# Fadi987/PL-BERT

Measured on AMD Instinct MI355X. Metric: phoneme-tokens/sec, higher is better.
Workload: dtype bf16; 1 GPU; PL-BERT masked-phoneme training step (fwd+loss+bwd+allreduce+AdamW), ALBERT hidden 768 / 12 shared layers / FFN 2048 / 12 heads, seq_len 512, batch 32 per GPU; global_batch=32, seq_len=512, parallelism=dp1

## Files before the change

include/plbert.h:

```cpp
#ifndef PLBERT_H
#define PLBERT_H

#include <stdint.h>

#ifdef __cplusplus
extern "C" {
#endif

typedef struct PlbEngine PlbEngine;

typedef struct {
  int32_t vocab_size;
  int32_t embedding_size;
  int32_t hidden_size;
  int32_t num_attention_heads;
  int32_t intermediate_size;
  int32_t num_hidden_layers;
  int32_t max_position_embeddings;
  int32_t type_vocab_size;
  float layer_norm_eps;
  int32_t num_phonemes;
  int32_t num_tokens;
  int32_t max_batch;
  int32_t max_seq;
// ... 210 lines not shown
int plb_profile_num_classes(void);
const char* plb_profile_class_name(int cls);
int plb_profile_read(double* ms, int64_t* launches, double* flops, double* bytes);

void plb_debug_skip_piece(int index);
void plb_debug_ln_fault(int mode, int launches);
int plb_debug_hb_audit(PlbEngine* e, int32_t on, int32_t break_wait);
int plb_debug_hb_report(const PlbEngine* e, int64_t* checks, int32_t* violations, char* first, int32_t first_bytes);
int plb_comm_trace(PlbEngine* e, int32_t on);
int plb_comm_trace_read(PlbEngine* e, int32_t max_pieces, int32_t* n, int64_t* begin, int64_t* end, float* released_ms,
                        float* done_ms, float* tail_ms);
void plb_set_gemm_nt_tile(int tile);
void plb_set_gemm_nt_prefetch(int on);
void plb_set_attn_bwd_fused(int on);
void plb_set_prune_last(int on);

#ifdef __cplusplus
}
#endif
#endif
```

plbert_amd/_lib.py:

```python
from __future__ import annotations

import ctypes as C
import os

import torch

HERE = os.path.dirname(os.path.abspath(__file__))
LIB_PATH = os.environ.get("PLBERT_HIP_LIB") or os.path.join(HERE, "libplbert_hip.so")

PLB_PARAM_NAMES = [
    "encoder.embeddings.word_embeddings.weight",
    "encoder.embeddings.position_embeddings.weight",
    "encoder.embeddings.token_type_embeddings.weight",
    "encoder.embeddings.LayerNorm.weight",
    "encoder.embeddings.LayerNorm.bias",
    "encoder.encoder.embedding_hidden_mapping_in.weight",
    "encoder.encoder.embedding_hidden_mapping_in.bias",
    "encoder.encoder.albert_layer_groups.0.albert_layers.0.full_layer_layer_norm.weight",
    "encoder.encoder.albert_layer_groups.0.albert_layers.0.full_layer_layer_norm.bias",
    "encoder.encoder.albert_layer_groups.0.albert_layers.0.attention.query.weight",
    "encoder.encoder.albert_layer_groups.0.albert_layers.0.attention.key.weight",
    "encoder.encoder.albert_layer_groups.0.albert_layers.0.attention.value.weight",
    "encoder.encoder.albert_layer_groups.0.albert_layers.0.attention.query.bias",
    "encoder.encoder.albert_layer_groups.0.albert_layers.0.attention.key.bias",
# ... 51 lines not shown


class PlbAttn(C.Structure):
    _fields_ = [
        ("qkv", C.c_void_p), ("ldqkv", C.c_int), ("lengths", C.c_void_p),
        ("B", C.c_int), ("S", C.c_int), ("NH", C.c_int), ("H", C.c_int), ("scale", C.c_float),
        ("ctx", C.c_void_p), ("ldctx", C.c_int), ("lse", C.c_void_p),
        ("dctx", C.c_void_p), ("lddctx", C.c_int), ("delta", C.c_void_p), ("dqkv", C.c_void_p), ("lddqkv", C.c_int),
        ("colpart", C.c_void_p), ("colpart_accumulate", C.c_int),
        ("ctx8", C.c_void_p), ("ldctx8", C.c_int), ("ctx_scale", C.c_void_p), ("ctx_amax", C.c_void_p),
        ("dqkv8", C.c_void_p), ("lddqkv8", C.c_int), ("dqkv_scale", C.c_void_p), ("dqkv_amax", C.c_void_p),
        ("qoff", C.c_void_p), ("q", C.c_void_p), ("ldq", C.c_int), ("nq_total", C.c_int), ("dq", C.c_void_p), ("lddq", C.c_int),
        ("dq8", C.c_void_p), ("lddq8", C.c_int),
        ("row_start", C.c_void_p),
        ("key_words", C.c_void_p), ("ldkw", C.c_int),
    ]


class PlbEmbed(C.Structure):
    _fields_ = [
        ("ids", C.c_void_p), ("T", C.c_int), ("S", C.c_int), ("E", C.c_int), ("V", C.c_int),
        ("word", C.c_void_p), ("pos", C.c_void_p), ("type0", C.c_void_p), ("gamma", C.c_void_p), ("beta", C.c_void_p),
        ("eps", C.c_float), ("out", C.c_void_p), ("ldo", C.c_int), ("dout", C.c_void_p), ("lddo", C.c_int),
        ("dx", C.c_void_p), ("dword", C.c_void_p), ("dpos", C.c_void_p), ("partials", C.c_void_p), ("nblocks", C.c_int),
        ("row_start", C.c_void_p), ("lengths", C.c_void_p), ("B", C.c_int), ("fill_slots", C.c_int),
    ]


class PlbEmbedIn(C.Structure):
    _fields_ = [
# ... 170 lines not shown
    "plb_mask_batch": (i32, [vp, vp, i32, i32, u64, u32, f32, f32, f32, i32, i32, vp, vp, vp, vp, vp]),
    "plb_profile_enable": (None, [i32]),
    "plb_profile_num_classes": (i32, []),
    "plb_profile_class_name": (C.c_char_p, [i32]),
    "plb_profile_read": (i32, [P(f64), P(i64), P(f64), P(f64)]),
    "plb_debug_skip_piece": (None, [i32]),
    "plb_debug_ln_fault": (None, [i32, i32]),
    "plb_debug_hb_audit": (i32, [vp, i32, i32]),
    "plb_debug_hb_report": (i32, [vp, P(i64), P(i32), vp, i32]),
    "plb_comm_trace": (i32, [vp, i32]),
    "plb_comm_trace_read": (i32, [vp, i32, P(i32), P(i64), P(i64), P(f32), P(f32), P(f32)]),
    "plb_set_gemm_nt_tile": (None, [i32]),
    "plb_set_gemm_nt_prefetch": (None, [i32]),
    "plb_set_attn_bwd_fused": (None, [i32]),
    "plb_set_prune_last": (None, [i32]),
}
PUBLIC_SYMBOLS = list(PUBLIC)
INTERNAL = {
    **{name: PUBLIC[name] for name in ("plb_set_gemm_nt_tile", "plb_set_gemm_nt_prefetch", "plb_debug_skip_piece",
                                       "plb_debug_ln_fault", "plb_set_attn_bwd_fused")},
    "plb_prof_begin": (i32, [i32, vp, f64, f64]),
    "plb_prof_end": (None, [i32, vp]),
    "plb_launch_gemm_nt_ln": (i32, [P(PlbGemmNT), i32, vp]),
    "plb_launch_gemm_nt_gelud": (i32, [P(PlbGemmNT), i32, vp]),
    "plb_launch_gemm_nt_fp8": (i32, [P(PlbGemmNT), i32, i32, vp]),
    "plb_launch_gemm_nt_fp8_ln": (i32, [P(PlbGemmNT), i32, i32, vp]),
    "plb_launch_gemm_nt_fp8_gelud": (i32, [P(PlbGemmNT), i32, i32, vp]),
    "plb_gemm_nt_fp8_gelud_tile_rows": (i32, [i32]),
    "plb_ln_fault_take": (i32, []),
    "plb_launch_gemm_nt": (i32, [P(PlbGemmNT), i32, i32, vp]),
# ... 11 lines not shown
    "plb_launch_embed_inputs_scatter": (i32, [P(PlbEmbedIn), vp]),
    "plb_embed_inputs_part_floats": (sz, [i32, i32, i32, i32]),
    "plb_launch_amax": (i32, [vp, i32, sz, i32, i32, vp, vp]),
    "plb_launch_fp8_scales": (i32, [vp, vp, vp, i32, f32, i32, vp]),
    "plb_launch_fp8_scales2": (i32, [vp, vp, vp, i32, f32, i32, i32, f32, vp, i32, vp]),
    "plb_launch_quantize": (i32, [vp, i32, sz, i32, i32, vp, vp, i32, i32, vp]),
    "plb_launch_quantize_multi": (i32, [i32, vp, vp, vp, vp, vp, vp, vp]),
    "plb_launch_ln_fwd": (i32, [P(PlbLayerNorm), vp]),
    "plb_launch_ln_bwd": (i32, [P(PlbLayerNorm), vp]),
    "plb_launch_colsum": (i32, [vp, i32, sz, i32, i32, vp, i32, i32, vp, i32, vp]),
    "plb_launch_copy_cols": (i32, [vp, i32, i32, i32, i32, vp, vp]),
    "plb_launch_pooler": (i32, [vp, i32, i32, i32, vp, vp, vp, vp]),
    "plb_launch_attn_fwd": (i32, [P(PlbAttn), vp]),
    "plb_launch_attn_bwd": (i32, [P(PlbAttn), vp]),
    "plb_launch_attn_bwd_fused": (i32, [P(PlbAttn), vp]),
    "plb_launch_gather_rows": (i32, [vp, i32, vp, i32, i32, i32, vp, i32, vp]),
    "plb_launch_scatter_rows": (i32, [vp, i32, vp, i32, i32, vp, i32, vp]),
    "plb_launch_ce_prepare": (i32, [vp, vp, vp, i32, i32, vp, vp, vp, vp]),
    "plb_launch_ce_prepare_packed": (i32, [vp, vp, vp, i32, i32, vp, vp, vp, vp, vp]),
    "plb_launch_unpack_rows": (i32, [vp, i32, i32, vp, vp, i32, i32, i32, vp, vp]),
    "plb_launch_seed_dy": (i32, [vp, vp, vp, i32, i32, i32, i32, vp, vp]),
    "plb_launch_pooler_bwd": (i32, [vp, i32, vp, i32, i32, i32, vp, vp, vp, vp, vp, vp, vp, vp]),
    "plb_launch_seed_dy_first_rows": (i32, [vp, vp, vp, i32, i32, i32, vp, vp]),
    "plb_launch_attn_probs": (i32, [vp, i32, vp, vp, vp, i32, i32, i32, f32, vp, vp]),
    "plb_launch_attn_probs_masked": (i32, [vp, i32, vp, vp, vp, vp, i32, i32, i32, i32, f32, vp, vp]),
    "plb_launch_key_mask_words": (i32, [vp, vp, i32, i32, vp, i32, vp]),
    "plb_launch_add_row_grad": (i32, [vp, vp, vp, vp, i32, i32, i32, i32, vp, vp]),
    "plb_launch_ce_fwd_bwd": (i32, [vp, i32, i32, vp, vp, i32, i32, vp, vp, i32, vp]),
    "plb_launch_sum_rows": (i32, [vp, i32, vp, vp]),
    "plb_launch_token_ce_combine": (i32, [vp, vp, i32, vp, vp, i32, i32, i32, vp, vp, vp, vp]),
# ... 81 lines not shown
```

plbert_amd/csrc/attn.hip:

```cpp
#include "attn_common.h"
#include <stdlib.h>
#include <string.h>

namespace {

#define ATTN_KM 0
#define ATTN_KERNEL(name) name##_kernel
#include "attn_kernels.h"
#undef ATTN_KM
#undef ATTN_KERNEL
#define ATTN_KM 1
#define ATTN_KERNEL(name) name##_km_kernel
#include "attn_kernels.h"
#undef ATTN_KM
#undef ATTN_KERNEL

}

static int check_attn(const PlbAttn* p) {
  if (p->H != p->NH * 64 || p->S < 1 || p->B < 1) return 1;
  if (p->row_start && !p->lengths) return 1;
  if (p->ldqkv % 8 || p->ldctx % 8) return 1;
  if (p->key_words && (p->S > 2048 || p->ldkw < 2 * ((p->S + 63) / 64) || p->qoff)) return 1;
  return 0;
}

extern "C" int plb_launch_attn_fwd(const PlbAttn* p, hipStream_t stream) {
  if (check_attn(p) || (p->ctx8 && (!p->ctx_scale || p->ldctx8 % 8))) return 1;
  if (p->qoff && (!p->q || p->ldq % 8 || p->nq_total < 0)) return 1;
  dim3 grid(((p->S + 127) / 128) * p->NH * p->B), block(256);
  const double unit = (double)p->B * p->NH * (double)p->S * p->S * 64.0;
  const double io = 2.0 * p->B * p->S * (double)p->H;
  const int tok = plb_prof_begin(PLB_K_ATTN_FWD, stream, 4.0 * unit, 4.0 * io);
  if (p->key_words) hipLaunchKernelGGL(attn_fwd_km_kernel, grid, block, 0, stream, *p);
  else hipLaunchKernelGGL(attn_fwd_kernel, grid, block, 0, stream, *p);
  plb_prof_end(tok, stream);
  return hipGetLastError() == hipSuccess ? 0 : 2;
}

static int g_bwd_fused = -2;
extern "C" void plb_set_attn_bwd_fused(int on) { g_bwd_fused = on < 0 ? -1 : (on > 2 ? 1 : on); }
static int launch_attn_bwd_split(const PlbAttn* p, hipStream_t stream) {
  dim3 grid(((p->S + 127) / 128) * p->NH * p->B), block(256);
  const double unit = (double)p->B * p->NH * (double)p->S * p->S * 64.0;
  const double io = 2.0 * p->B * p->S * (double)p->H;
  int tok = plb_prof_begin(PLB_K_ATTN_BWD_DQ, stream, 4.0 * unit, 6.0 * io);
  if (p->key_words) hipLaunchKernelGGL(attn_bwd_dq_km_kernel, grid, block, 0, stream, *p);
  else hipLaunchKernelGGL(attn_bwd_dq_kernel, grid, block, 0, stream, *p);
  plb_prof_end(tok, stream);
  tok = plb_prof_begin(PLB_K_ATTN_BWD_DKV, stream, 4.0 * unit, 6.0 * io);
  if (p->key_words) hipLaunchKernelGGL(attn_bwd_dkv_km_kernel, grid, block, 0, stream, *p);
  else hipLaunchKernelGGL(attn_bwd_dkv_kernel, grid, block, 0, stream, *p);
  plb_prof_end(tok, stream);
  return hipGetLastError() == hipSuccess ? 0 : 2;
}
static PlbAttn attn_samples(const PlbAttn* p, int b0, int nb) {
  PlbAttn q = *p;
  const size_t t0 = (size_t)b0 * p->S;
  q.B = nb;
// ... 2 lines not shown
  q.dctx = p->dctx + t0 * p->lddctx;
  if (p->dqkv) q.dqkv = p->dqkv + t0 * p->lddqkv;
  if (p->dqkv8) q.dqkv8 = p->dqkv8 + t0 * p->lddqkv8;
  if (p->lengths) q.lengths = p->lengths + b0;
  q.lse = p->lse + (size_t)b0 * p->NH * p->S;
  if (p->delta) q.delta = p->delta + (size_t)b0 * p->NH * p->S;
  if (p->colpart) q.colpart = p->colpart + (size_t)b0 * ((p->S + 127) / 128) * 4 * (3 * p->H);
  if (p->key_words) q.key_words = p->key_words + (size_t)b0 * p->ldkw;
  if (p->row_start) {
    q.row_start = p->row_start + b0;
    q.qkv = p->qkv; q.ctx = p->ctx; q.dctx = p->dctx; q.dqkv = p->dqkv; q.dqkv8 = p->dqkv8;
  }
  return q;
}

extern "C" int plb_launch_attn_bwd(const PlbAttn* p, hipStream_t stream) {
  if (check_attn(p) || p->lddctx % 8 || p->lddqkv % 8 || (!p->dqkv && !p->dqkv8) || (p->dqkv8 && (!p->dqkv_scale || p->lddqkv8 % 8))) return 1;
  if (g_bwd_fused == -2) {
    const char* e = getenv("PLBERT_ATTN_BWD");
    g_bwd_fused = (e && !strcmp(e, "fused")) ? 1 : (e && !strcmp(e, "split")) ? 0 : (e && !strcmp(e, "hybrid")) ? 2 : -1;
  }
  const bool hybrid_on = g_bwd_fused == 2;
  if (p->qoff && (!p->q || p->ldq % 8 || p->nq_total < 0 || (!p->dq && !p->dq8) || (p->dq && p->lddq % 8) || (p->dq8 && p->lddq8 % 8))) return 1;
  const bool can_fuse = p->S <= 512 && !(p->dqkv && p->dqkv8) && !p->qoff && !p->key_words;
  if (!can_fuse || g_bwd_fused == 0) return launch_attn_bwd_split(p, stream);
  if (g_bwd_fused == 1) return plb_launch_attn_bwd_fused(p, stream);
  if (p->S <= 384) return launch_attn_bwd_split(p, stream);
  const int items = p->B * p->NH, rounds = (items + 255) / 256;
  if (items * 10 >= rounds * 256 * 9) return plb_launch_attn_bwd_fused(p, stream);
  const int per_round = 256 / p->NH;
  const int full = per_round > 0 ? (p->B / per_round) : 0;
  const int nb_f = full * per_round, rest = p->B - nb_f;
  if (hybrid_on && full >= 1 && per_round * p->NH * 10 >= 256 * 9 && rest * p->NH <= 160) {
    const PlbAttn a = attn_samples(p, 0, nb_f);
    const int rc = plb_launch_attn_bwd_fused(&a, stream);
    if (rc || rest == 0) return rc;
    const PlbAttn b = attn_samples(p, nb_f, rest);
    return launch_attn_bwd_split(&b, stream);
  }
  return launch_attn_bwd_split(p, stream);
}
```

plbert_amd/csrc/attn_kernels.h:

```cpp
#define KEY_WORDS(kwl_, kt_)                                                                                       \
  uint32_t kw0 = ~0u, kw1 = ~0u;                                                                                   \
  if constexpr (ATTN_KM) {                                                                                              \
    kw0 = (uint32_t)__builtin_amdgcn_readlane((int)(kwl_), 2 * (kt_));                                             \
    kw1 = (uint32_t)__builtin_amdgcn_readlane((int)(kwl_), 2 * (kt_) + 1);                                         \
  }

#ifndef RESCALE_TH
#define RESCALE_TH 8.0f
#endif
#ifndef FWD_WAVES
#define FWD_WAVES 3
#endif
__global__ __launch_bounds__(256, ATTN_KM ? 4 : FWD_WAVES) void ATTN_KERNEL(attn_fwd)(PlbAttn p) {
  __shared__ __attribute__((aligned(16))) bf16_t smem[2][2][64 * 64];
  const int tid = threadIdx.x, lane = tid & 63;
  const int wave = __builtin_amdgcn_readfirstlane(tid >> 6);
  DBG_EARLY_EXIT(p);
  const int QT = (p.S + 127) >> 7;
  const int logical = xcd_remap(blockIdx.x, gridDim.x);
  const int bx = logical % QT, bh = logical / QT;
  const int hd = bh % p.NH, b = bh / p.NH;
  const int S = p.S, H = p.H;
  int len = p.lengths ? p.lengths[b] : S;
  len = len < 1 ? 1 : (len > S ? S : len);
// ... 474 lines not shown
  float* cp = p.colpart ? p.colpart + ((size_t)(b * QT + bx) * 4 + wave) * (3 * H) + hd * 64 : nullptr;
  int lane_e = (int)__builtin_amdgcn_mbcnt_hi(~0u, __builtin_amdgcn_mbcnt_lo(~0u, 0u));
  asm volatile("" : "+v"(lane_e));
  float amax8 = 0.f;
  if (rows_valid > 0) {
    bf16_t* out = p.dqkv ? p.dqkv + (tok0 + key0) * p.lddqkv + hd * 64 : nullptr;
    uint8_t* out8 = p.dqkv8 ? p.dqkv8 + (tok0 + key0) * p.lddqkv8 + hd * 64 : nullptr;
    const float qs8 = p.dqkv8 ? p.dqkv_scale[0] : 1.0f;
    const Out8 ok8 = {out8 ? out8 + H : nullptr, p.lddqkv8, qs8, true}, ov8 = {out8 ? out8 + 2 * H : nullptr, p.lddqkv8, qs8, true};
    const bool accq = p.colpart_accumulate != 0;
    store_transposed<(ATTN_OUT_NT & 4) != 0, true>(dk0, dk1, p.scale, patch, out ? out + H : nullptr, p.lddqkv, rows_valid, lane_e,
                                             cp ? cp + H : nullptr, accq, &ok8, &amax8);
    __builtin_amdgcn_wave_barrier();
    store_transposed<(ATTN_OUT_NT & 4) != 0, true>(dv0, dv1, 1.0f, patch, out ? out + 2 * H : nullptr, p.lddqkv, rows_valid, lane_e,
                                             cp ? cp + 2 * H : nullptr, accq, &ov8, &amax8);
  } else if (cp && !p.colpart_accumulate) {
    cp[H + lane_e] = 0.f;
    cp[2 * H + lane_e] = 0.f;
  }
  if (p.dqkv8 && p.dqkv_amax) {
    amax8 = wave_max(amax8);
    if (lane_e == 0) atomic_max_abs(p.dqkv_amax, amax8, blockIdx.x * 4 + wave);
  }
}
#undef KEY_WORDS
```

plbert_amd/csrc/engine_calls.cpp:

```cpp
#include "engine_internal.h"

void drop_stash(PlbEngine* e, const char* by) {
  if (e && e->stash_live) { e->stash_live = false; e->stash_dead_by = by; }
}

void drop_final(PlbEngine* e, const char* by) {
  if (e) { e->fin_live = false; e->fin_dead_by = by; }
}
static void note_final(PlbEngine* e, const bf16_t* x, const Call& c) {
  e->fin_live = true; e->fin_x = x; e->fin_B = c.B; e->fin_S = c.S;
  e->fin_rows = c.rw.Tp; e->fin_used = c.rw.T; e->fin_row_start = c.rw.row_start;
}

static int check_shape(const PlbEngine* e, int B, int S, const char* who) {
  if (!e || !e->ws) return fail("%s: engine not bound", who);
  if (B < 1 || S < 1 || B > e->c.max_batch || S > e->c.max_seq || (int64_t)B * S > (int64_t)e->c.max_batch * e->c.max_seq)
    return fail("%s: batch %d x seq %d exceeds the engine capacity %d x %d", who, B, S, e->c.max_batch, e->c.max_seq);
  return 0;
}

static Rows padded_rows(int B, int S) { return Rows{nullptr, B * S, rup(B * S, 128)}; }
static int pick_rows(PlbEngine* e, const PlbPacking* pk, const int32_t* lengths, bool padded, int B, int S, const char* who,
                     Rows* out) {
  *out = padded_rows(B, S);
// ... 388 lines not shown
  Rows rw;
  if (pick_rows(e, pk, lengths, token_targets != nullptr && !e->packed_dual, B, S, who, &rw)) return 1;
  const int64_t Tp = rw.Tp;
  e->rep_valid = false;
  e->rep_n = n_masked; e->rep_B = B; e->rep_dual = token_targets != nullptr; e->rep_tok_rows = token_targets ? Tp : 0;
  const Call c = {who, masked_ids, lengths, B, S, rw, {}, nullptr, s};
  if (backward && begin_training_call(e, token_targets != nullptr, s)) return 1;
  if (n_masked == 0 && !token_targets) {
    drop_final(e, "the last loss call had no masked position and no token targets: it did not run the encoder");
    if (zero_loss_call(e, backward, loss, s)) return 1;
    e->rep_valid = true;
    return 0;
  }

  const int NM = (int)rup(n_masked, 128);
  Prune pr = {e->at<int32_t>(e->o_rows), n_masked, NM};
  const bool prune = prune_enabled() && n_masked > 0 && !token_targets && e->L >= 2 && 2 * (int64_t)NM <= Tp;
  if (n_masked > 0) {
    if (rw.row_start)
      TRY(plb_launch_ce_prepare_packed(idx_offsets, idx_flat, labels, B, S, rw.row_start, e->at<int32_t>(e->o_rows),
                                       e->at<int32_t>(e->o_tgt), e->at<float>(e->o_w), s));
    else
      TRY(plb_launch_ce_prepare(idx_offsets, idx_flat, labels, B, S, e->at<int32_t>(e->o_rows), e->at<int32_t>(e->o_tgt),
                                e->at<float>(e->o_w), s));
  }
  if (backward) e->pruned_rows = prune ? NM : 0;
  e->last_app_rows[0] = prune ? NM : Tp; e->last_app_rows[1] = Tp;
  bf16_t* xL = nullptr;
  if (run_encoder(e, c, backward, &xL, prune ? &pr : nullptr)) return 1;
  bf16_t* dy = backward ? e->at<bf16_t>(e->o_dy0) : nullptr;
  if (phoneme_head(e, backward, prune, xL, n_masked, Tp, dy, loss, s)) return 1;
  if (loss_parts) HIPTRY(hipMemcpyAsync(loss_parts, loss, sizeof(float), hipMemcpyDeviceToDevice, s));
// ... 223 lines not shown
```

plbert_amd/csrc/engine_internal.h:

```cpp
#pragma once
#include <hip/hip_runtime.h>
#include <stdint.h>
#include <stdio.h>
#include <stdlib.h>
#include <string.h>

#include <array>
#include <map>
#include <string>
#include <vector>

#include "../../include/plbert.h"
#include "plbert_kernels.h"

#pragma GCC visibility push(hidden)

int fail(const char* fmt, ...);

static const unsigned kStreamOrderEvent = hipEventDisableTiming | hipEventReleaseToDevice;

inline int64_t rup(int64_t x, int64_t m) { return (x + m - 1) / m * m; }

#define TRY(x)                                                                    \
  do {                                                                            \
// ... 164 lines not shown

struct F8Op { const uint8_t* A8; const uint8_t* B8; const float* deq_a; const float* deq_b; int a_bf8; };

struct Slots {
  bf16_t *x, *y;
  bf16_t *qkv, *ctx, *pre1, *a, *u, *g, *pre2;
  float *mean1, *rstd1, *mean2, *rstd2, *lse;
  uint8_t *x8, *x8n, *c8, *a8, *g8;
  bf16_t *dqkv, *dpre1, *du, *dpre2;
  uint8_t *dp8, *du8, *dp18, *dq8;
  float *part1, *part2, *qkvcol, *ducol;
};

struct LnSlot { const float* gamma; const float* beta; const bf16_t* pre; float* mean; float* rstd; float* partials; };

struct Prune { const int32_t* rows; int n; int Mc; };

struct EmbedCall {
  PlbEmbedInputs in;
  float* d_inputs_embeds;
  bool any() const { return in.token_type_ids || in.position_ids || in.inputs_embeds || d_inputs_embeds; }
};

struct Call {
  const char* who;
  const int64_t* ids;
  const int32_t* lengths;
  int B, S;
  Rows rw;
  EmbedCall ec;
  const PlbLayerOutputs* taps;
// ... 20 lines not shown
int64_t piece_begin(const PlbEngine* e, int i);
int64_t piece_end(const PlbEngine* e, int i);
int reduce_pieces(PlbEngine* e, int from, int to, hipStream_t after);
int status_exchange(PlbEngine* e, hipStream_t s);
int status_finish(PlbEngine* e, float* loss, hipStream_t s);
int f8_site(const PlbEngine* e, int site, int l);
float* f8_deq(const PlbEngine* e, int i);
int fp8_quantize_weights(PlbEngine* e, hipStream_t s, bool exact = true);
int fp8_update_scales(PlbEngine* e, hipStream_t s);
bool f8_call(const PlbEngine* e, int64_t Tp, bool train);
bool tn8_ok(const PlbEngine* e, int64_t Mtot);
PlbGemmNT nt_desc(const bf16_t* A, const bf16_t* B, int64_t M, int N, int K);
int qkvcol_rows(int B, int S);
Slots slots(const PlbEngine* e, int64_t Tp, int B, int S, int l, bool stash, int prows = 0, int du_rows = 0);
bool prune_enabled();
int run_encoder(PlbEngine* e, const Call& c, bool stash, bf16_t** xout, const Prune* pr);
PlbEmbed embed_desc(const PlbEngine* e, const Call& c);
PlbEmbedIn embed_in_desc(const PlbEngine* e, const EmbedCall& ec, const PlbEmbed* base);
int tn_splits(int64_t Mtot, int N, int K, int* rows_per_split);
int weight_grad(PlbEngine* e, const bf16_t* A, int lda, int Ncols, const bf16_t* Bm, int ldb, int64_t Mtot, int N,
                int K, float* out, hipStream_t s, bool side_slab = false);
int weight_grad8(PlbEngine* e, const uint8_t* A8, const uint8_t* B8, int64_t Mtot, int N, int K, int site_a, int site_b,
                 float* out, hipStream_t s);
int encoder_bwd(PlbEngine* e, const Call& c, const Prune* pr, bf16_t** dy, int* du_rows, const float* const* d_below);
void drop_stash(PlbEngine* e, const char* by);
void drop_final(PlbEngine* e, const char* by);
int sync_transposes(PlbEngine* e, hipStream_t s, bool exact_fp8 = true);
inline int64_t pool_end(const PlbEngine* e) { return e->poff[PLB_POOL_B] + e->psize[PLB_POOL_B]; }
void end_accum_window(PlbEngine* e, const char* by);

// ... 2 lines not shown
```

plbert_amd/csrc/engine_layers.cpp:

```cpp
#include "engine_internal.h"

static bool tn_big(int64_t Mtot, int Ncols, int K) { return Ncols % 256 == 0 && K % 256 == 0 && Mtot >= 8192; }
static bool tn_fill_chip() {
  static const bool v = [] { const char* e = getenv("PLBERT_TN_SPLITS"); return !(e && !strcmp(e, "xcd")); }();
  return v;
}
static int tn_cus() {
  static const int v = [] {
    const char* e = getenv("PLBERT_TN_CUS");
    const int n = e ? atoi(e) : 256;
    return (n >= 64 && n <= 256) ? n : 256;
  }();
  return v;
}
int tn_splits(int64_t Mtot, int N, int K, int* rows_per_split) {
  const bool big = tn_big(Mtot, N, K);
  const int tiles = big ? (N / 256) * (K / 256) : ((N + 127) / 128) * ((K + 127) / 128);
  int splits = 768 / tiles;
  if (big) {
    int s = 32 / tiles;
    if (s < 1) s = 1;
    splits = tiles >= 256 ? 1 : (tn_fill_chip() ? (tn_cus() / tiles > 0 ? tn_cus() / tiles : 1) : 8 * s);
  }
  const int64_t maxs = Mtot / 64;
// ... 118 lines not shown
    ln_fields(e, g, ln.gamma, nullptr, ln.mean, ln.rstd);
    if (dx8) f8_out(g, dx8, e->H, q, 1);
    TRY(gemm_nt_ln_any(g, 6, f8, s));
    return 0;
  }
  TRY(gemm_nt_any(g, 0, f8, s));
  return ln_bwd(e, ln, nblocks, g->C, dx, T, Tzero, dx8, q, s);
}

static int g_prune_last = -1;
extern "C" void plb_set_prune_last(int on) { g_prune_last = on < 0 ? -1 : (on ? 1 : 0); }
bool prune_enabled() {
  static const bool v = [] { const char* e = getenv("PLBERT_PRUNE_LAST"); return !(e && !strcmp(e, "0")); }();
  return g_prune_last < 0 ? v : g_prune_last != 0;
}
static int last_application_fwd_pruned(PlbEngine* e, const Prune* pr, bool stash, bool calib, bool tn8, const Slots& sl,
                                       const bf16_t* ctx_att, hipStream_t s) {
  const int H = e->H, I = e->I, L = e->L, Mc = pr->Mc, n = pr->n;
  const F8Site sA(e, F8_A, L - 1), sG(e, F8_G, L - 1), sC(e, F8_C, L - 1);
  bf16_t* ctxc = stash ? sl.ctx : sl.pre1;
  bf16_t* xc = stash ? e->at<bf16_t>(e->o_da) : sl.a;
  bf16_t* pre1c = stash ? sl.pre1 : sl.ctx;
  bf16_t* ac = stash ? sl.a : sl.pre1;
  TRY(plb_launch_gather_rows(ctx_att, H, pr->rows, n, Mc, H, ctxc, H, s));
  TRY(plb_launch_gather_rows(sl.x, H, pr->rows, n, Mc, H, xc, H, s));
  PlbGemmNT g = nt_desc(ctxc, e->wbf(PLB_DENSE_W), Mc, H, H);
  g.bias = e->par(PLB_DENSE_B); g.res = xc; g.ldr = H; g.C = pre1c; g.ldc = H;
  const LnSlot ln1 = {e->par(PLB_LN1_W), e->par(PLB_LN1_B), pre1c, sl.mean1, sl.rstd1, nullptr};
  if (gemm_ln_fwd(e, &g, nullptr, false, ln1, ac, Mc, nullptr, F8Site(), s)) return 1;
  if (calib) TRY(plb_launch_amax(ac, 1, (size_t)n, H, H, sA.amax, s));
  g = nt_desc(ac, e->wbf(PLB_FFN_W), Mc, I, H);
  g.bias = e->par(PLB_FFN_B); g.C = sl.u; g.ldc = I; g.C2 = sl.g; g.ldc2 = I;
  TRY(plb_launch_gemm_nt(&g, 1, 0, s));
  if (calib) TRY(plb_launch_amax(sl.g, 1, (size_t)n, I, I, sG.amax, s));
  g = nt_desc(sl.g, e->wbf(PLB_FFNO_W), Mc, H, I);
  g.bias = e->par(PLB_FFNO_B); g.res = ac; g.ldr = H; g.C = sl.pre2; g.ldc = H;
  if (gemm_ln_fwd(e, &g, nullptr, false, ln2_slot(e, sl), e->at<bf16_t>(e->o_hm), Mc, nullptr, F8Site(), s)) return 1;
  if (tn8) {
    const void* src[3] = {ctxc, ac, sl.g}; const int fl[3] = {1, 1, 1};
    const size_t nel[3] = {(size_t)Mc * H, (size_t)Mc * H, (size_t)Mc * I};
    const float* sc[3] = {sC.scale, sA.scale, sG.scale};
    uint8_t* dst[3] = {sl.c8, sl.a8, sl.g8};
    float* am[3] = {sC.amax, sA.amax, sG.amax};
    TRY(plb_launch_quantize_multi(3, src, fl, nel, sc, dst, am, s));
  }
  return 0;
}

static int tap_hidden(PlbEngine* e, const Call& c, int slot, const bf16_t* x) {
  float* const out = (c.taps && c.taps->hidden_states) ? c.taps->hidden_states[slot] : nullptr;
  if (!out) return 0;
  if (c.lengths) TRY(plb_launch_unpack_rows(x, 1, e->H, c.rw.row_start, c.lengths, c.B, c.S, e->H, out, c.s));
  else TRY(plb_launch_bf16_to_f32(x, e->H, out, e->H, c.rw.T, e->H, c.s));
  return 0;
}

PlbEmbed embed_desc(const PlbEngine* e, const Call& c) {
  PlbEmbed em;
  memset(&em, 0, sizeof(em));
  em.ids = c.ids; em.T = c.rw.T; em.S = c.S; em.E = e->E; em.V = e->V;
  em.word = e->par(PLB_WORD_EMB); em.pos = e->par(PLB_POS_EMB); em.type0 = e->par(PLB_TYPE_EMB);
  em.gamma = e->par(PLB_EMB_LN_W); em.beta = e->par(PLB_EMB_LN_B); em.eps = e->c.layer_norm_eps;
  if (c.rw.row_start) { em.row_start = c.rw.row_start; em.lengths = c.lengths; em.B = c.B; }
// ... 39 lines not shown
  if (f8) {
    const F8Site sX(e, F8_X, 0);
    const void* src1[1] = {first.x}; const int bf1[1] = {1}; const size_t n1[1] = {(size_t)T8 * H};
    const float* sc1[1] = {sX.scale}; uint8_t* dst1[1] = {first.x8}; float* am1[1] = {sX.amax};
    TRY(plb_launch_quantize_multi(1, src1, bf1, n1, sc1, dst1, am1, s));
  }
  const bool fuse_f = ln_fusable(e, Tp, 1);
  const bool dstash = gelu_dstash(e, Tp, f8);
  if (stash) e->tn8_call = f8 && e->fp8_tn && dstash && tn8_ok(e, (int64_t)L * Tp);
  const bool tn8 = stash && e->tn8_call;

  for (int l = 0; l < L; ++l) {
    const Slots sl = slots(e, Tp, B, S, l, stash);
    const F8Site sX(e, F8_X, l), sA(e, F8_A, l), sG(e, F8_G, l), sC(e, F8_C, l);
    if (calib) TRY(plb_launch_amax(sl.x, 1, (size_t)T, H, H, sX.amax, s));
    g = nt_desc(sl.x, e->wbf(PLB_Q_W), Tp, 3 * H, H);
    g.bias = e->par(PLB_Q_B); g.C = sl.qkv; g.ldc = 3 * H;
    const F8Op oq = f8_op(sl.x8, sX, F8Weight(e, F8W_QKV), 0);
    TRY(gemm_nt_any(&g, 0, f8 ? &oq : nullptr, s));
    PlbAttn at;
    memset(&at, 0, sizeof(at));
    at.qkv = sl.qkv; at.ldqkv = 3 * H; at.lengths = c.lengths; at.B = B; at.S = S; at.NH = e->NH; at.H = H;
    at.row_start = rw.row_start;
    at.key_words = rw.key_words; at.ldkw = rw.ldkw;
    const bool pruned_layer = pr != nullptr && l == L - 1;
    bf16_t* const ctx_att = (pruned_layer && stash) ? e->at<bf16_t>(e->o_dy1) : sl.ctx;
    at.scale = 0.125f; at.ctx = ctx_att; at.ldctx = H; at.lse = sl.lse;
    if (f8 && !pruned_layer) { at.ctx8 = sl.c8; at.ldctx8 = H; at.ctx_scale = sC.scale; at.ctx_amax = sC.amax; }
    if (rw.row_start && e->fp8_on && S % 128) {
      HIPTRY(hipMemsetAsync(ctx_att, 0, (size_t)T * H * 2, s));
// ... 134 lines not shown
  g = nt_desc(sl.du, e->at<bf16_t>(e->o_w1T), Mc, H, I);
  g.res = sl.dpre2; g.ldr = H; g.C = dac; g.ldc = H;
  if (gemm_ln_bwd(e, &g, nullptr, false, ln1_slot(e, sl), c.prows, sl.dpre1, Mc, Mc, nullptr, F8Site(), s)) return 1;
  if (c.calib) TRY(plb_launch_amax(sl.dpre1, 1, (size_t)n, H, H, sDP1.amax, s));
  if (e->tn8_call) {
    const void* src[3] = {sl.dpre2, sl.du, sl.dpre1}; const int fl[3] = {3, 3, 3};
    const size_t nel[3] = {(size_t)Mc * H, (size_t)Mc * I, (size_t)Mc * H};
    const float* sc[3] = {sDP.scale, sDU.scale, sDP1.scale};
    uint8_t* dst[3] = {sl.dp8, sl.du8, sl.dp18};
    float* am[3] = {sDP.amax, sDU.amax, sDP1.amax};
    TRY(plb_launch_quantize_multi(3, src, fl, nel, sc, dst, am, s));
  }
  g = nt_desc(sl.dpre1, e->at<bf16_t>(e->o_wdT), Mc, H, H);
  g.C = dctxc; g.ldc = H;
  TRY(plb_launch_gemm_nt(&g, 0, 0, s));
  HIPTRY(hipMemsetAsync(dctx, 0, (size_t)Tp * H * 2, s));
  TRY(plb_launch_scatter_rows(dctxc, H, pr->rows, n, H, dctx, H, s));
  HIPTRY(hipMemsetAsync(dac, 0, (size_t)Tp * H * 2, s));
  TRY(plb_launch_scatter_rows(sl.dpre1, H, pr->rows, n, H, dac, H, s));
  return 0;
}

static int attention_bwd_dx(PlbEngine* e, const Bwd& c, int l, const Slots& sl, bf16_t* ctx, const bf16_t* res,
                            bf16_t* dx, const float* d_in) {
  const Call& call = c.call;
  const Rows& rw = call.rw;
  const int H = e->H, T = rw.T;
  const int64_t Tp = rw.Tp;
  hipStream_t s = call.s;
  if (d_in) {
    bf16_t* const res_in = e->at<bf16_t>(e->o_da);
    HB_R(s, res, Tp * H * 2, "residual operand of the dX GEMM");
    HB_W(s, res_in, Tp * H * 2, "residual operand + the caller's gradient of this application's input");
    TRY(plb_launch_add_row_grad(res, d_in, call.lengths, rw.row_start, call.B, call.S, H, (int)Tp, res_in, s));
    res = res_in;
  }
  const F8Site sDQ(e, F8_DQ, l);
  PlbAttn at;
  memset(&at, 0, sizeof(at));
  at.qkv = sl.qkv; at.ldqkv = 3 * H; at.lengths = call.lengths; at.B = call.B; at.S = call.S; at.NH = e->NH; at.H = H; at.scale = 0.125f;
  at.row_start = rw.row_start;
  at.key_words = rw.key_words; at.ldkw = rw.ldkw;
  at.ctx = ctx; at.ldctx = H; at.lse = sl.lse;
  at.dctx = e->at<bf16_t>(e->o_dctx); at.lddctx = H; at.delta = e->at<float>(e->o_delta); at.dqkv = sl.dqkv; at.lddqkv = 3 * H;
  at.colpart = sl.qkvcol; at.colpart_accumulate = 0;
  if (c.f8) {
    at.dqkv8 = sl.dq8; at.lddqkv8 = 3 * H; at.dqkv_scale = sDQ.scale; at.dqkv_amax = sDQ.amax;
    if (e->tn8_call) at.dqkv = nullptr;
  }
  if (rw.row_start && call.S % 128 && at.dqkv) HIPTRY(hipMemsetAsync(sl.dqkv, 0, (size_t)T * 3 * H * 2, s));
  if (rw.row_start && call.S % 128 && at.dqkv8) HIPTRY(hipMemsetAsync(sl.dq8, 0, (size_t)T * 3 * H, s));
  TRY(plb_launch_attn_bwd(&at, s));
  if (Tp > T) {
    if (at.dqkv) HIPTRY(hipMemsetAsync(sl.dqkv + (int64_t)T * 3 * H, 0, (size_t)(Tp - T) * 3 * H * 2, s));
    if (c.f8) HIPTRY(hipMemsetAsync(sl.dq8 + (int64_t)T * 3 * H, 0, (size_t)(Tp - T) * 3 * H, s));
  }
  if (c.calib) TRY(plb_launch_amax(sl.dqkv, 1, (size_t)T, 3 * H, 3 * H, sDQ.amax, s));
  PlbGemmNT g = nt_desc(sl.dqkv, e->at<bf16_t>(e->o_wqkvT), Tp, H, 3 * H);
  g.res = res; g.ldr = H; g.C = dx; g.ldc = H;
  const F8Op ox = f8_op(sl.dq8, sDQ, F8Weight(e, F8W_QKVT), 1);
  if (l == 0) {
    TRY(gemm_nt_any(&g, 0, c.f8 ? &ox : nullptr, s));
    return 0;
  }
  const Slots below = slots(e, Tp, call.B, call.S, l - 1, true, c.prows, c.du_rows);
  return gemm_ln_bwd(e, &g, c.f8 ? &ox : nullptr, c.fuse_b, ln2_slot(e, below), c.prows, below.dpre2, T, (int)Tp,
                     c.f8 ? below.dp8 : nullptr, F8Site(e, F8_DP, l - 1), s);
// ... 3 lines not shown
  const int I = e->I, L = e->L;
  Bwd c = {call};
  const int Tp = (int)call.rw.Tp;
  c.f8 = f8_call(e, Tp, true);
  c.calib = e->fp8_on && !c.f8;
  c.du_rows = e->u_is_derivative ? (c.f8 ? 2 * (Tp / plb_gemm_nt_fp8_gelud_tile_rows(Tp)) : 2 * (Tp / 256))
                                 : (c.f8 ? 2 * (Tp / 128) : plb_gemm_nt_colpart_rows(Tp, I, e->H));
  c.fuse_b = ln_fusable(e, Tp, 2);
  c.prows = c.fuse_b ? 2 * Tp / 128 : e->ln_blocks;
  e->part_rows_used = c.prows;
  bf16_t* dx = e->at<bf16_t>(e->o_dy1);
  for (int l = L - 1; l >= 0; --l) {
    const Slots sl = slots(e, call.rw.Tp, call.B, call.S, l, true, c.prows, c.du_rows);
    if (pr && l == L - 1) {
      if (last_application_bwd_pruned(e, c, sl, pr)) return 1;
      if (attention_bwd_dx(e, c, l, sl, e->at<bf16_t>(e->o_dy1), e->at<bf16_t>(e->o_da), dx, nullptr)) return 1;
    } else {
      if (post_attention_bwd(e, c, l, sl, *dy)) return 1;
      if (attention_bwd_dx(e, c, l, sl, sl.ctx, sl.dpre1, dx, d_below ? d_below[l] : nullptr)) return 1;
    }
    bf16_t* tmp = *dy; *dy = dx; dx = tmp;
  }
  *du_rows = c.du_rows;
  return 0;
}
```

plbert_amd/csrc/plbert_kernels.h:

```cpp
#pragma once
#include <hip/hip_runtime.h>
#include <stdint.h>

#include "../../include/plbert.h"

typedef uint16_t bf16_t;

extern "C" {

enum PlbKernelClass {
  PLB_K_GEMM_NT = 0, PLB_K_GEMM_NT_GELU, PLB_K_GEMM_NT_GELUBWD, PLB_K_GEMM_NT_F32, PLB_K_GEMM_TN,
  PLB_K_ATTN_FWD, PLB_K_ATTN_BWD_DQ, PLB_K_ATTN_BWD_DKV, PLB_K_LN_FWD, PLB_K_LN_BWD, PLB_K_EMBED_FWD,
  PLB_K_EMBED_BWD, PLB_K_COLSUM, PLB_K_REDUCE, PLB_K_ROWS, PLB_K_CE, PLB_K_ADAMW, PLB_K_CAST, PLB_K_TOKEN_CE, PLB_K_GEMM_NT_CE, PLB_K_GEMM_NT_SMALL, PLB_K_FP8, PLB_K_ATTN_BWD,
  PLB_K_GEMM_NT_FP8, PLB_K_GEMM_NT_GELU_FP8, PLB_K_GEMM_NT_GELUBWD_FP8,
  PLB_K_GEMM_NT_LNFWD, PLB_K_GEMM_NT_LNBWD,
  PLB_K_GEMM_NT_LNFWD_FP8, PLB_K_GEMM_NT_LNBWD_FP8, PLB_K_GEMM_TN_FP8,
  PLB_K_NCLASS
};
int plb_prof_begin(int cls, hipStream_t s, double flops, double bytes);
void plb_prof_end(int tok, hipStream_t s);

typedef struct {
  const bf16_t* A; int lda;
  const bf16_t* B; int ldb;
// ... 119 lines not shown
  const int32_t* lengths;
  int B, S, NH, H;
  float scale;
  bf16_t* ctx; int ldctx;
  float* lse;
  const bf16_t* dctx; int lddctx;
  float* delta;
  bf16_t* dqkv; int lddqkv;
  float* colpart;
  int colpart_accumulate;
  uint8_t* ctx8; int ldctx8; const float* ctx_scale; float* ctx_amax;
  uint8_t* dqkv8; int lddqkv8; const float* dqkv_scale; float* dqkv_amax;
  const int32_t* qoff; const bf16_t* q; int ldq; int nq_total; bf16_t* dq; int lddq; uint8_t* dq8; int lddq8;
  const int32_t* row_start;
  const uint32_t* key_words; int ldkw;
} PlbAttn;
int plb_launch_attn_fwd(const PlbAttn* p, hipStream_t stream);
int plb_launch_attn_bwd(const PlbAttn* p, hipStream_t stream);
int plb_launch_attn_bwd_fused(const PlbAttn* p, hipStream_t stream);
void plb_debug_skip_piece(int index);
void plb_debug_ln_fault(int mode, int launches);
void plb_set_attn_bwd_fused(int on);

int plb_launch_gather_rows(const bf16_t* src, int lds_, const int32_t* rows, int n, int npad, int H, bf16_t* dst,
                           int ldd, hipStream_t stream);
int plb_launch_scatter_rows(const bf16_t* src, int lds_, const int32_t* rows, int n, int H, bf16_t* dst, int ldd,
                            hipStream_t stream);
int plb_launch_ce_prepare(const int32_t* offsets, const int32_t* flat, const int64_t* labels, int B, int S,
                          int32_t* rows, int32_t* tgt, float* w, hipStream_t stream);
int plb_launch_ce_prepare_packed(const int32_t* offsets, const int32_t* flat, const int64_t* labels, int B, int S,
                                 const int32_t* row_start, int32_t* rows, int32_t* tgt, float* w, hipStream_t stream);
int plb_launch_unpack_rows(const void* src, int src_is_bf16, int lds_, const int32_t* row_start, const int32_t* lengths,
                           int B, int S, int C, float* dst, hipStream_t stream);
int plb_launch_seed_dy(const float* d_hidden, const int32_t* lengths, const int32_t* row_start, int B, int S, int H, int Tp,
// ... 108 lines not shown
```

Baseline: 1.757 million tokens/s.

## Prune last-layer attention to masked query rows in forward and backward

In the last encoder layer, only masked positions feed the loss. The change computes Q projections and attention only for the masked query rows, while K/V are still computed for every token. Backward runs attention with a compact query set, zeroes the Q block of dqkv and scatters dq back into place. This drops the row gathers and the dctx scatter for that layer. It applies only when the split backward form is selected and FP8 and key-mask paths are off, and it adds more path complexity.

```diff
diff --git a/include/plbert.h b/include/plbert.h
--- a/include/plbert.h
+++ b/include/plbert.h
@@ -248,6 +248,7 @@
 void plb_set_gemm_nt_prefetch(int on);
 void plb_set_attn_bwd_fused(int on);
 void plb_set_prune_last(int on);
+void plb_set_prune_attn(int on);
 
 #ifdef __cplusplus
 }
diff --git a/plbert_amd/_lib.py b/plbert_amd/_lib.py
--- a/plbert_amd/_lib.py
+++ b/plbert_amd/_lib.py
@@ -89,6 +89,7 @@
         ("dq8", C.c_void_p), ("lddq8", C.c_int),
         ("row_start", C.c_void_p),
         ("key_words", C.c_void_p), ("ldkw", C.c_int),
+        ("zero_q_block", C.c_int),
     ]
 
 
@@ -289,6 +290,7 @@
     "plb_set_gemm_nt_prefetch": (None, [i32]),
     "plb_set_attn_bwd_fused": (None, [i32]),
     "plb_set_prune_last": (None, [i32]),
+    "plb_set_prune_attn": (None, [i32]),
 }
 PUBLIC_SYMBOLS = list(PUBLIC)
 INTERNAL = {
@@ -330,6 +332,7 @@
     "plb_launch_attn_fwd": (i32, [P(PlbAttn), vp]),
     "plb_launch_attn_bwd": (i32, [P(PlbAttn), vp]),
     "plb_launch_attn_bwd_fused": (i32, [P(PlbAttn), vp]),
+    "plb_attn_bwd_form": (i32, [P(PlbAttn)]),
     "plb_launch_gather_rows": (i32, [vp, i32, vp, i32, i32, i32, vp, i32, vp]),
     "plb_launch_scatter_rows": (i32, [vp, i32, vp, i32, i32, vp, i32, vp]),
     "plb_launch_ce_prepare": (i32, [vp, vp, vp, i32, i32, vp, vp, vp, vp]),
diff --git a/plbert_amd/csrc/attn.hip b/plbert_amd/csrc/attn.hip
--- a/plbert_amd/csrc/attn.hip
+++ b/plbert_amd/csrc/attn.hip
@@ -22,14 +22,19 @@
   if (p->row_start && !p->lengths) return 1;
   if (p->ldqkv % 8 || p->ldctx % 8) return 1;
   if (p->key_words && (p->S > 2048 || p->ldkw < 2 * ((p->S + 63) / 64) || p->qoff)) return 1;
+  if (p->zero_q_block && !p->qoff) return 1;
   return 0;
+}
+
+static double attn_unit(const PlbAttn* p) {
+  return (p->qoff ? (double)p->NH * p->nq_total : (double)p->B * p->NH * p->S) * (double)p->S * 64.0;
 }
 
 extern "C" int plb_launch_attn_fwd(const PlbAttn* p, hipStream_t stream) {
   if (check_attn(p) || (p->ctx8 && (!p->ctx_scale || p->ldctx8 % 8))) return 1;
   if (p->qoff && (!p->q || p->ldq % 8 || p->nq_total < 0)) return 1;
   dim3 grid(((p->S + 127) / 128) * p->NH * p->B), block(256);
-  const double unit = (double)p->B * p->NH * (double)p->S * p->S * 64.0;
+  const double unit = attn_unit(p);
   const double io = 2.0 * p->B * p->S * (double)p->H;
   const int tok = plb_prof_begin(PLB_K_ATTN_FWD, stream, 4.0 * unit, 4.0 * io);
   if (p->key_words) hipLaunchKernelGGL(attn_fwd_km_kernel, grid, block, 0, stream, *p);
@@ -42,7 +47,7 @@
 extern "C" void plb_set_attn_bwd_fused(int on) { g_bwd_fused = on < 0 ? -1 : (on > 2 ? 1 : on); }
 static int launch_attn_bwd_split(const PlbAttn* p, hipStream_t stream) {
   dim3 grid(((p->S + 127) / 128) * p->NH * p->B), block(256);
-  const double unit = (double)p->B * p->NH * (double)p->S * p->S * 64.0;
+  const double unit = attn_unit(p);
   const double io = 2.0 * p->B * p->S * (double)p->H;
   int tok = plb_prof_begin(PLB_K_ATTN_BWD_DQ, stream, 4.0 * unit, 6.0 * io);
   if (p->key_words) hipLaunchKernelGGL(attn_bwd_dq_km_kernel, grid, block, 0, stream, *p);
@@ -75,29 +80,34 @@
   return q;
 }
 
-extern "C" int plb_launch_attn_bwd(const PlbAttn* p, hipStream_t stream) {
-  if (check_attn(p) || p->lddctx % 8 || p->lddqkv % 8 || (!p->dqkv && !p->dqkv8) || (p->dqkv8 && (!p->dqkv_scale || p->lddqkv8 % 8))) return 1;
+extern "C" int plb_attn_bwd_form(const PlbAttn* p) {
   if (g_bwd_fused == -2) {
     const char* e = getenv("PLBERT_ATTN_BWD");
     g_bwd_fused = (e && !strcmp(e, "fused")) ? 1 : (e && !strcmp(e, "split")) ? 0 : (e && !strcmp(e, "hybrid")) ? 2 : -1;
   }
-  const bool hybrid_on = g_bwd_fused == 2;
-  if (p->qoff && (!p->q || p->ldq % 8 || p->nq_total < 0 || (!p->dq && !p->dq8) || (p->dq && p->lddq % 8) || (p->dq8 && p->lddq8 % 8))) return 1;
   const bool can_fuse = p->S <= 512 && !(p->dqkv && p->dqkv8) && !p->qoff && !p->key_words;
-  if (!can_fuse || g_bwd_fused == 0) return launch_attn_bwd_split(p, stream);
-  if (g_bwd_fused == 1) return plb_launch_attn_bwd_fused(p, stream);
-  if (p->S <= 384) return launch_attn_bwd_split(p, stream);
+  if (!can_fuse || g_bwd_fused == 0) return 0;
+  if (g_bwd_fused == 1) return 1;
+  if (p->S <= 384) return 0;
   const int items = p->B * p->NH, rounds = (items + 255) / 256;
-  if (items * 10 >= rounds * 256 * 9) return plb_launch_attn_bwd_fused(p, stream);
+  if (items * 10 >= rounds * 256 * 9) return 1;
   const int per_round = 256 / p->NH;
   const int full = per_round > 0 ? (p->B / per_round) : 0;
-  const int nb_f = full * per_round, rest = p->B - nb_f;
-  if (hybrid_on && full >= 1 && per_round * p->NH * 10 >= 256 * 9 && rest * p->NH <= 160) {
-    const PlbAttn a = attn_samples(p, 0, nb_f);
-    const int rc = plb_launch_attn_bwd_fused(&a, stream);
-    if (rc || rest == 0) return rc;
-    const PlbAttn b = attn_samples(p, nb_f, rest);
-    return launch_attn_bwd_split(&b, stream);
-  }
-  return launch_attn_bwd_split(p, stream);
+  if (g_bwd_fused == 2 && full >= 1 && per_round * p->NH * 10 >= 256 * 9 && (p->B - full * per_round) * p->NH <= 160) return 2;
+  return 0;
 }
+
+extern "C" int plb_launch_attn_bwd(const PlbAttn* p, hipStream_t stream) {
+  if (check_attn(p) || p->lddctx % 8 || p->lddqkv % 8 || (!p->dqkv && !p->dqkv8) || (p->dqkv8 && (!p->dqkv_scale || p->lddqkv8 % 8))) return 1;
+  if (p->qoff && (!p->q || p->ldq % 8 || p->nq_total < 0 || (!p->dq && !p->dq8) || (p->dq && p->lddq % 8) || (p->dq8 && p->lddq8 % 8))) return 1;
+  if (p->zero_q_block && !p->dqkv) return 1;
+  const int form = plb_attn_bwd_form(p);
+  if (form == 0) return launch_attn_bwd_split(p, stream);
+  if (form == 1) return plb_launch_attn_bwd_fused(p, stream);
+  const int nb_f = (p->B / (256 / p->NH)) * (256 / p->NH), rest = p->B - nb_f;
+  const PlbAttn a = attn_samples(p, 0, nb_f);
+  const int rc = plb_launch_attn_bwd_fused(&a, stream);
+  if (rc || rest == 0) return rc;
+  const PlbAttn b = attn_samples(p, nb_f, rest);
+  return launch_attn_bwd_split(&b, stream);
+}
diff --git a/plbert_amd/csrc/attn_kernels.h b/plbert_amd/csrc/attn_kernels.h
--- a/plbert_amd/csrc/attn_kernels.h
+++ b/plbert_amd/csrc/attn_kernels.h
@@ -512,6 +512,13 @@
     __builtin_amdgcn_wave_barrier();
     store_transposed<(ATTN_OUT_NT & 4) != 0, true>(dv0, dv1, 1.0f, patch, out ? out + 2 * H : nullptr, p.lddqkv, rows_valid, lane_e,
                                              cp ? cp + 2 * H : nullptr, accq, &ov8, &amax8);
+    if (p.zero_q_block && p.qoff && out) {
+#pragma unroll
+      for (int i = 0; i < 4; ++i) {
+        const int id = lane_e + 64 * i, row = id >> 3, c = id & 7;
+        if (row < rows_valid) *(uint4*)(out + (size_t)row * p.lddqkv + c * 8) = make_uint4(0u, 0u, 0u, 0u);
+      }
+    }
   } else if (cp && !p.colpart_accumulate) {
     cp[H + lane_e] = 0.f;
     cp[2 * H + lane_e] = 0.f;
diff --git a/plbert_amd/csrc/engine_calls.cpp b/plbert_amd/csrc/engine_calls.cpp
--- a/plbert_amd/csrc/engine_calls.cpp
+++ b/plbert_amd/csrc/engine_calls.cpp
@@ -426,8 +426,9 @@
   }
 
   const int NM = (int)rup(n_masked, 128);
-  Prune pr = {e->at<int32_t>(e->o_rows), n_masked, NM};
+  Prune pr = {e->at<int32_t>(e->o_rows), n_masked, NM, nullptr};
   const bool prune = prune_enabled() && n_masked > 0 && !token_targets && e->L >= 2 && 2 * (int64_t)NM <= Tp;
+  if (prune && prune_attn_ok(e, c, backward)) pr.qoff = idx_offsets;
   if (n_masked > 0) {
     if (rw.row_start)
       TRY(plb_launch_ce_prepare_packed(idx_offsets, idx_flat, labels, B, S, rw.row_start, e->at<int32_t>(e->o_rows),
diff --git a/plbert_amd/csrc/engine_internal.h b/plbert_amd/csrc/engine_internal.h
--- a/plbert_amd/csrc/engine_internal.h
+++ b/plbert_amd/csrc/engine_internal.h
@@ -202,7 +202,7 @@
 
 struct LnSlot { const float* gamma; const float* beta; const bf16_t* pre; float* mean; float* rstd; float* partials; };
 
-struct Prune { const int32_t* rows; int n; int Mc; };
+struct Prune { const int32_t* rows; int n; int Mc; const int32_t* qoff; };
 
 struct EmbedCall {
   PlbEmbedInputs in;
@@ -253,6 +253,7 @@
 int qkvcol_rows(int B, int S);
 Slots slots(const PlbEngine* e, int64_t Tp, int B, int S, int l, bool stash, int prows = 0, int du_rows = 0);
 bool prune_enabled();
+bool prune_attn_ok(const PlbEngine* e, const Call& c, bool train);
 int run_encoder(PlbEngine* e, const Call& c, bool stash, bf16_t** xout, const Prune* pr);
 PlbEmbed embed_desc(const PlbEngine* e, const Call& c);
 PlbEmbedIn embed_in_desc(const PlbEngine* e, const EmbedCall& ec, const PlbEmbed* base);
diff --git a/plbert_amd/csrc/engine_layers.cpp b/plbert_amd/csrc/engine_layers.cpp
--- a/plbert_amd/csrc/engine_layers.cpp
+++ b/plbert_amd/csrc/engine_layers.cpp
@@ -156,6 +156,17 @@
   static const bool v = [] { const char* e = getenv("PLBERT_PRUNE_LAST"); return !(e && !strcmp(e, "0")); }();
   return g_prune_last < 0 ? v : g_prune_last != 0;
 }
+static int g_prune_attn = -1;
+extern "C" void plb_set_prune_attn(int on) { g_prune_attn = on < 0 ? -1 : (on ? 1 : 0); }
+bool prune_attn_ok(const PlbEngine* e, const Call& c, bool train) {
+  static const bool v = [] { const char* s = getenv("PLBERT_PRUNE_ATTN"); return !(s && !strcmp(s, "0")); }();
+  if (!(g_prune_attn < 0 ? v : g_prune_attn != 0)) return false;
+  if (c.rw.key_words || f8_call(e, c.rw.Tp, train)) return false;
+  PlbAttn full;
+  memset(&full, 0, sizeof(full));
+  full.B = c.B; full.S = c.S; full.NH = e->NH; full.H = e->H; full.dqkv = e->at<bf16_t>(e->o_dqkv);
+  return plb_attn_bwd_form(&full) == 0;
+}
 static int last_application_fwd_pruned(PlbEngine* e, const Prune* pr, bool stash, bool calib, bool tn8, const Slots& sl,
                                        const bf16_t* ctx_att, hipStream_t s) {
   const int H = e->H, I = e->I, L = e->L, Mc = pr->Mc, n = pr->n;
@@ -164,8 +175,10 @@
   bf16_t* xc = stash ? e->at<bf16_t>(e->o_da) : sl.a;
   bf16_t* pre1c = stash ? sl.pre1 : sl.ctx;
   bf16_t* ac = stash ? sl.a : sl.pre1;
-  TRY(plb_launch_gather_rows(ctx_att, H, pr->rows, n, Mc, H, ctxc, H, s));
-  TRY(plb_launch_gather_rows(sl.x, H, pr->rows, n, Mc, H, xc, H, s));
+  if (!pr->qoff) {
+    TRY(plb_launch_gather_rows(ctx_att, H, pr->rows, n, Mc, H, ctxc, H, s));
+    TRY(plb_launch_gather_rows(sl.x, H, pr->rows, n, Mc, H, xc, H, s));
+  }
   PlbGemmNT g = nt_desc(ctxc, e->wbf(PLB_DENSE_W), Mc, H, H);
   g.bias = e->par(PLB_DENSE_B); g.res = xc; g.ldr = H; g.C = pre1c; g.ldc = H;
   const LnSlot ln1 = {e->par(PLB_LN1_W), e->par(PLB_LN1_B), pre1c, sl.mean1, sl.rstd1, nullptr};
@@ -189,6 +202,31 @@
   return 0;
 }
 
+static int attention_fwd_compact(PlbEngine* e, const Call& c, const Prune* pr, bool stash, bool calib, const Slots& sl) {
+  const int H = e->H, L = e->L, Mc = pr->Mc, n = pr->n;
+  const int64_t Tp = c.rw.Tp;
+  hipStream_t s = c.s;
+  bf16_t* ctxc = stash ? sl.ctx : sl.pre1;
+  bf16_t* xc = stash ? e->at<bf16_t>(e->o_da) : sl.a;
+  TRY(plb_launch_gather_rows(sl.x, H, pr->rows, n, Mc, H, xc, H, s));
+  PlbGemmNT g = nt_desc(sl.x, e->wbf(PLB_Q_W) + (int64_t)H * H, Tp, 2 * H, H);
+  g.bias = e->par(PLB_Q_B) + H; g.C = sl.qkv + H; g.ldc = 3 * H;
+  TRY(plb_launch_gemm_nt(&g, 0, 0, s));
+  g = nt_desc(xc, e->wbf(PLB_Q_W), Mc, H, H);
+  g.bias = e->par(PLB_Q_B); g.C = sl.qkv; g.ldc = 3 * H;
+  TRY(plb_launch_gemm_nt(&g, 0, 0, s));
+  PlbAttn at;
+  memset(&at, 0, sizeof(at));
+  at.qkv = sl.qkv; at.ldqkv = 3 * H; at.lengths = c.lengths; at.B = c.B; at.S = c.S; at.NH = e->NH; at.H = H; at.scale = 0.125f;
+  at.row_start = c.rw.row_start;
+  at.qoff = pr->qoff; at.q = sl.qkv; at.ldq = 3 * H; at.nq_total = n;
+  at.ctx = ctxc; at.ldctx = H; at.lse = sl.lse;
+  TRY(plb_launch_attn_fwd(&at, s));
+  if (Mc > n) HIPTRY(hipMemsetAsync(ctxc + (int64_t)n * H, 0, (size_t)(Mc - n) * H * 2, s));
+  if (calib) TRY(plb_launch_amax(ctxc, 1, (size_t)n, H, H, F8Site(e, F8_C, L - 1).amax, s));
+  return 0;
+}
+
 static int tap_hidden(PlbEngine* e, const Call& c, int slot, const bf16_t* x) {
   float* const out = (c.taps && c.taps->hidden_states) ? c.taps->hidden_states[slot] : nullptr;
   if (!out) return 0;
@@ -258,6 +296,12 @@
     const Slots sl = slots(e, Tp, B, S, l, stash);
     const F8Site sX(e, F8_X, l), sA(e, F8_A, l), sG(e, F8_G, l), sC(e, F8_C, l);
     if (calib) TRY(plb_launch_amax(sl.x, 1, (size_t)T, H, H, sX.amax, s));
+    if (pr && pr->qoff && l == L - 1) {
+      if (attention_fwd_compact(e, c, pr, stash, calib, sl)) return 1;
+      if (last_application_fwd_pruned(e, pr, stash, calib, tn8, sl, nullptr, s)) return 1;
+      *xout = e->at<bf16_t>(e->o_hm);
+      break;
+    }
     g = nt_desc(sl.x, e->wbf(PLB_Q_W), Tp, 3 * H, H);
     g.bias = e->par(PLB_Q_B); g.C = sl.qkv; g.ldc = 3 * H;
     const F8Op oq = f8_op(sl.x8, sX, F8Weight(e, F8W_QKV), 0);
@@ -422,15 +466,17 @@
   g = nt_desc(sl.dpre1, e->at<bf16_t>(e->o_wdT), Mc, H, H);
   g.C = dctxc; g.ldc = H;
   TRY(plb_launch_gemm_nt(&g, 0, 0, s));
-  HIPTRY(hipMemsetAsync(dctx, 0, (size_t)Tp * H * 2, s));
-  TRY(plb_launch_scatter_rows(dctxc, H, pr->rows, n, H, dctx, H, s));
+  if (!pr->qoff) {
+    HIPTRY(hipMemsetAsync(dctx, 0, (size_t)Tp * H * 2, s));
+    TRY(plb_launch_scatter_rows(dctxc, H, pr->rows, n, H, dctx, H, s));
+  }
   HIPTRY(hipMemsetAsync(dac, 0, (size_t)Tp * H * 2, s));
   TRY(plb_launch_scatter_rows(sl.dpre1, H, pr->rows, n, H, dac, H, s));
   return 0;
 }
 
 static int attention_bwd_dx(PlbEngine* e, const Bwd& c, int l, const Slots& sl, bf16_t* ctx, const bf16_t* res,
-                            bf16_t* dx, const float* d_in) {
+                            bf16_t* dx, const float* d_in, const Prune* cq = nullptr) {
   const Call& call = c.call;
   const Rows& rw = call.rw;
   const int H = e->H, T = rw.T;
@@ -452,6 +498,11 @@
   at.ctx = ctx; at.ldctx = H; at.lse = sl.lse;
   at.dctx = e->at<bf16_t>(e->o_dctx); at.lddctx = H; at.delta = e->at<float>(e->o_delta); at.dqkv = sl.dqkv; at.lddqkv = 3 * H;
   at.colpart = sl.qkvcol; at.colpart_accumulate = 0;
+  if (cq) {
+    at.qoff = cq->qoff; at.q = sl.qkv; at.ldq = 3 * H; at.nq_total = cq->n;
+    at.dctx = e->at<bf16_t>(e->o_dy0);
+    at.dq = e->at<bf16_t>(e->o_dctx); at.lddq = H; at.zero_q_block = 1;
+  }
   if (c.f8) {
     at.dqkv8 = sl.dq8; at.lddqkv8 = 3 * H; at.dqkv_scale = sDQ.scale; at.dqkv_amax = sDQ.amax;
     if (e->tn8_call) at.dqkv = nullptr;
@@ -459,6 +510,7 @@
   if (rw.row_start && call.S % 128 && at.dqkv) HIPTRY(hipMemsetAsync(sl.dqkv, 0, (size_t)T * 3 * H * 2, s));
   if (rw.row_start && call.S % 128 && at.dqkv8) HIPTRY(hipMemsetAsync(sl.dq8, 0, (size_t)T * 3 * H, s));
   TRY(plb_launch_attn_bwd(&at, s));
+  if (cq) TRY(plb_launch_scatter_rows(at.dq, H, cq->rows, cq->n, H, sl.dqkv, 3 * H, s));
   if (Tp > T) {
     if (at.dqkv) HIPTRY(hipMemsetAsync(sl.dqkv + (int64_t)T * 3 * H, 0, (size_t)(Tp - T) * 3 * H * 2, s));
     if (c.f8) HIPTRY(hipMemsetAsync(sl.dq8 + (int64_t)T * 3 * H, 0, (size_t)(Tp - T) * 3 * H, s));
@@ -492,7 +544,9 @@
     const Slots sl = slots(e, call.rw.Tp, call.B, call.S, l, true, c.prows, c.du_rows);
     if (pr && l == L - 1) {
       if (last_application_bwd_pruned(e, c, sl, pr)) return 1;
-      if (attention_bwd_dx(e, c, l, sl, e->at<bf16_t>(e->o_dy1), e->at<bf16_t>(e->o_da), dx, nullptr)) return 1;
+      if (attention_bwd_dx(e, c, l, sl, pr->qoff ? sl.ctx : e->at<bf16_t>(e->o_dy1), e->at<bf16_t>(e->o_da), dx, nullptr,
+                           pr->qoff ? pr : nullptr))
+        return 1;
     } else {
       if (post_attention_bwd(e, c, l, sl, *dy)) return 1;
       if (attention_bwd_dx(e, c, l, sl, sl.ctx, sl.dpre1, dx, d_below ? d_below[l] : nullptr)) return 1;
diff --git a/plbert_amd/csrc/plbert_kernels.h b/plbert_amd/csrc/plbert_kernels.h
--- a/plbert_amd/csrc/plbert_kernels.h
+++ b/plbert_amd/csrc/plbert_kernels.h
@@ -157,10 +157,12 @@
   const int32_t* qoff; const bf16_t* q; int ldq; int nq_total; bf16_t* dq; int lddq; uint8_t* dq8; int lddq8;
   const int32_t* row_start;
   const uint32_t* key_words; int ldkw;
+  int zero_q_block;
 } PlbAttn;
 int plb_launch_attn_fwd(const PlbAttn* p, hipStream_t stream);
 int plb_launch_attn_bwd(const PlbAttn* p, hipStream_t stream);
 int plb_launch_attn_bwd_fused(const PlbAttn* p, hipStream_t stream);
+int plb_attn_bwd_form(const PlbAttn* p);
 void plb_debug_skip_piece(int index);
 void plb_debug_ln_fault(int mode, int launches);
 void plb_set_attn_bwd_fused(int on);
```

After: 1.775 million tokens/s (median of 6 runs). 1.01x the previous value.
